# ParthaEth/GIF

Hardware: NVIDIA H100
Metric: G+D train step images/sec @256x256 bs32/GPU (higher is better)
Workload: dtype bf16x3 error-compensated tensor-core contraction (two-term bf16 operands, 3 MMAs per slice), f32 accumulate/storage

## Files before the change

### gif_b200/_lib.py

```python
import ctypes
import os

import torch

_HERE = os.path.dirname(os.path.abspath(__file__))
LIB_PATH = os.path.join(_HERE, "libgifb200.so")

_p = ctypes.c_void_p
_i = ctypes.c_int
_f = ctypes.c_float
_d = ctypes.c_double
_ll = ctypes.c_longlong
_sz = ctypes.c_size_t

SIGNATURES = {
    "gifb200_version": (_i, []),
    "gifb200_last_error": (ctypes.c_char_p, []),
    "gifb200_launch_count": (_ll, []),
    "gifb200_conv2d_workspace_bytes": (_sz, [_i] * 11),
    "gifb200_conv2d": (_i, [_p, _p, _p] + [_i] * 13 + [_p, _f, _f, _i, _p, _sz, _p]),
    "gifb200_conv2d_wgrad_workspace_bytes": (_sz, [_i] * 10),
    "gifb200_conv2d_wgrad_path": (_i, [_i] * 10),
    "gifb200_conv2d_wgrad": (_i, [_p, _p, _p] + [_i] * 12 + [_p, _sz, _p]),
    "gifb200_conv2d_ex_workspace_bytes": (_sz, [_i] * 13),
    "gifb200_conv2d_ex": (_i, [_p, _p, _p] + [_i] * 16 + [_p, _i, _p, _sz, _p]),
    "gifb200_pool2d": (_i, [_p, _p] + [_i] * 12 + [_p]),
    "gifb200_resize_bilinear": (_i, [_p, _p, _i, _i, _i, _ll, _ll, _ll, _ll, _i, _i, _i, _f, _f, _i, _p]),
    "gifb200_resize_bilinear_u8": (_i, [_p, _p, _i, _i, _i, _ll, _i, _i, _i, _f, _f, _i, _p]),
    "gifb200_split_bf16": (_i, [_p, _p, _p, _i, _i, _i, _p]),
    "gifb200_upfirdn2d": (_i, [_p, _p, _p] + [_i] * 14 + [_p]),
    "gifb200_bias_act": (_i, [_p, _p, _p, _p, _p, _i, _i, _i, _f, _f, _i, _p]),
    "gifb200_act_bwd": (_i, [_p, _p, _p, _ll, _f, _f, _i, _p]),
    "gifb200_rows_sum": (_i, [_p, _p, _i, _i, _i, _p]),
    "gifb200_chan_scale": (_i, [_p, _p, _p, _i, _i, _i, _i, _p]),
    "gifb200_tail_bwd": (_i, [_p] * 8 + [_i, _i, _i, _f, _f, _i, _p]),
    "gifb200_tail_bwd_planes": (_i, [_p] * 8 + [_i, _i, _i, _f, _f, _p, _p, _p]),
    "gifb200_scale_bwd": (_i, [_p] * 5 + [_i, _i, _i, _i, _p]),
    "gifb200_tail_bwd2": (_i, [_p] * 9 + [_i, _i, _i, _f, _f, _p, _p]),
    "gifb200_adam_step": (_i, [_p, _p, _p, _p, _p, _p, _i, _d, _d, _d, _d, _p]),
    "gifb200_spatial_dot": (_i, [_p, _p, _p, _i, _i, _i, _p]),
    "gifb200_axpby": (_i, [_p, _p, _p, _ll, _f, _f, _i, _p]),
    "gifb200_demod": (_i, [_p, _p, _p, _i, _i, _i, _f, _p]),
    "gifb200_torgb_fwd": (_i, [_p, _p, _p, _i, _i, _i, _p]),
    "gifb200_torgb_bwd_x": (_i, [_p, _p, _p, _i, _i, _i, _p]),
    "gifb200_torgb_bwd_w": (_i, [_p, _p, _p, _i, _i, _i, _p]),
    "gifb200_sgemm": (_i, [_i, _i, _i, _i, _i, _f, _p, _i, _p, _i, _p, _i, _p]),
    "gifb200_cond_down": (_i, [_p, _p, _i, _i, _i, _i, _i, _i, _p]),
    "gifb200_cond_up": (_i, [_p, _p, _i, _i, _i, _i, _i, _i, _p]),
    "gifb200_rasterize_workspace_bytes": (_sz, [_i, _i, _i, _i]),
    "gifb200_rasterize_fwd": (_i, [_p, _p, _p, _p, _p, _i, _i, _i, _i, _p, _sz, _p]),
    "gifb200_rasterize_fwd_ex": (_i, [_p] * 7 + [_i] * 5 + [_p, _sz, _p]),
    "gifb200_rasterize_bwd_ex": (_i, [_p] * 11 + [_i] * 5 + [_p]),
    "gifb200_render_shade": (_i, [_p] * 10 + [_i] * 5 + [_p]),
    "gifb200_vertex_normals": (_i, [_p] * 6 + [_i] * 3 + [_p]),
    "gifb200_rasterize_bwd": (_i, [_p, _p, _p, _p, _p, _p, _p, _p, _i, _i, _i, _i, _p]),
    "gifb200_flame_lbs_workspace_bytes": (_sz, [_i, _i]),
    "gifb200_flame_lbs": (_i, [_p] * 11 + [_i] * 4 + [_p, _sz, _p]),
    "gifb200_eye_camera": (_i, [_p, _p] + [_i] * 4 + [_f] * 4 + [_p]),
    "gifb200_flametex": (_i, [_p] * 4 + [_i] * 4 + [_p]),
    "gifb200_texture_steal_fwd": (_i, [_p] * 9 + [_i] * 6 + [_p]),
    "gifb200_texture_steal_bwd": (_i, [_p] * 7 + [_i] * 6 + [_p]),
    "gifb200_jpeg_workspace_bytes": (_sz, [_i, _i, _ll]),
    "gifb200_jpeg_decode": (_i, [_p] * 6 + [_i, _i, _i, _ll, _i, _i, _p, _p, _p, _sz, _p]),
    "gifb200_png_unfilter": (_i, [_p, _p, _i, _i, _p, _p, _p]),
    "gifb200_resize_bicubic_u8": (_i, [_p] * 5 + [_i] * 7 + [_p]),
    "gifb200_u8_to_unit": (_i, [_p, _p, _i, _i, _i, _ll, _p]),
    "gifb200_image_to_u8": (_i, [_p, _p, _i, _i, _i, _ll, _ll, _ll, _ll, _p]),
}


def _bind(path):
    lib = ctypes.CDLL(path)
    for name, (res, args) in SIGNATURES.items():
        fn = getattr(lib, name)
        fn.restype = res
        fn.argtypes = args
    return lib


def _load():
    import importlib.util
    spec = importlib.util.spec_from_file_location("_gifb200_build", os.path.join(_HERE, "build.py"))
# ... 39 lines not shown
```

### gif_b200/csrc/elementwise.cu

```cuda
#include <cuda_bf16.h>

#include <mutex>

#include "common.cuh"

namespace gifb200 {

thread_local char g_err[512] = "";
long long g_launches = 0;

template <bool VEC>
__global__ void __launch_bounds__(256) bias_act_kernel(const float* __restrict__ x, const float* __restrict__ rowscale,
                                                       const float* __restrict__ add, const float* __restrict__ bias,
                                                       float* __restrict__ y, long long total, int P, int C, float slope,
                                                       float gain, int rtf32) {
    const long long stride = static_cast<long long>(gridDim.x) * blockDim.x;
    if (VEC) {
        const long long nvec = total >> 2;
        const int c4n = C >> 2;
        for (long long v = static_cast<long long>(blockIdx.x) * blockDim.x + threadIdx.x; v < nvec; v += stride) {
            const int c = static_cast<int>(v % c4n) << 2;
            float4 t = __ldcs(reinterpret_cast<const float4*>(x) + v);
            if (rowscale) {
                const long long b = (v / c4n) / P;
// ... 374 lines not shown
                                                         float* __restrict__ y, long long total, int P, int C,
                                                         int rtf32) {
    const long long stride = static_cast<long long>(gridDim.x) * blockDim.x;
    if (VEC) {
        const long long nvec = total >> 2;
        const int c4n = C >> 2;
        for (long long v = static_cast<long long>(blockIdx.x) * blockDim.x + threadIdx.x; v < nvec; v += stride) {
            const int c = static_cast<int>(v % c4n) << 2;
            const long long b = (v / c4n) / P;
            float4 t = __ldcs(reinterpret_cast<const float4*>(x) + v);
            const float4 sc = *reinterpret_cast<const float4*>(s + b * C + c);
            t.x *= sc.x; t.y *= sc.y; t.z *= sc.z; t.w *= sc.w;
            if (rtf32) { t.x = round_tf32(t.x); t.y = round_tf32(t.y); t.z = round_tf32(t.z); t.w = round_tf32(t.w); }
            reinterpret_cast<float4*>(y)[v] = t;
        }
    } else {
        for (long long i = static_cast<long long>(blockIdx.x) * blockDim.x + threadIdx.x; i < total; i += stride) {
            float t = x[i] * s[((i / C) / P) * C + (i % C)];
            y[i] = rtf32 ? round_tf32(t) : t;
        }
    }
}


__global__ void __launch_bounds__(256) split_bf16_kernel(const float* __restrict__ x, const float* __restrict__ s,
                                                         __nv_bfloat16* __restrict__ planes, long long total, int P, int C) {
    const long long stride = static_cast<long long>(gridDim.x) * blockDim.x;
    const long long nvec = total >> 2;
    const int c4n = C >> 2;
    __nv_bfloat16* hi = planes;
    __nv_bfloat16* lo = planes + total;
    for (long long v = static_cast<long long>(blockIdx.x) * blockDim.x + threadIdx.x; v < nvec; v += stride) {
        float4 t = __ldcs(reinterpret_cast<const float4*>(x) + v);
        if (s) {
            const int c = static_cast<int>(v % c4n) << 2;
            const long long b = (v / c4n) / P;
            const float4 sc = *reinterpret_cast<const float4*>(s + b * C + c);
            t.x *= sc.x; t.y *= sc.y; t.z *= sc.z; t.w *= sc.w;
        }
        const __nv_bfloat16 h0 = __float2bfloat16_rn(t.x), h1 = __float2bfloat16_rn(t.y), h2 = __float2bfloat16_rn(t.z),
                            h3 = __float2bfloat16_rn(t.w);
        const __nv_bfloat16 l0 = __float2bfloat16_rn(t.x - __bfloat162float(h0)), l1 = __float2bfloat16_rn(t.y - __bfloat162float(h1)),
                            l2 = __float2bfloat16_rn(t.z - __bfloat162float(h2)), l3 = __float2bfloat16_rn(t.w - __bfloat162float(h3));
        uint2 ph, pl;
        ph.x = static_cast<uint32_t>(__bfloat16_as_ushort(h0)) | (static_cast<uint32_t>(__bfloat16_as_ushort(h1)) << 16);
        ph.y = static_cast<uint32_t>(__bfloat16_as_ushort(h2)) | (static_cast<uint32_t>(__bfloat16_as_ushort(h3)) << 16);
        pl.x = static_cast<uint32_t>(__bfloat16_as_ushort(l0)) | (static_cast<uint32_t>(__bfloat16_as_ushort(l1)) << 16);
        pl.y = static_cast<uint32_t>(__bfloat16_as_ushort(l2)) | (static_cast<uint32_t>(__bfloat16_as_ushort(l3)) << 16);
        reinterpret_cast<uint2*>(hi)[v] = ph;
        reinterpret_cast<uint2*>(lo)[v] = pl;
    }
}

template <bool VEC>
__global__ void __launch_bounds__(256) axpby_kernel(const float* __restrict__ a, const float* __restrict__ b,
                                                    float* __restrict__ y, long long n, float alpha, float beta,
                                                    int rtf32) {
    const long long stride = static_cast<long long>(gridDim.x) * blockDim.x;
    if (VEC) {
        const long long nvec = n >> 2;
        for (long long v = static_cast<long long>(blockIdx.x) * blockDim.x + threadIdx.x; v < nvec; v += stride) {
            float4 t = __ldcs(reinterpret_cast<const float4*>(a) + v);
            t.x *= alpha; t.y *= alpha; t.z *= alpha; t.w *= alpha;
            if (b) {
                const float4 u = __ldcs(reinterpret_cast<const float4*>(b) + v);
                t.x += beta * u.x; t.y += beta * u.y; t.z += beta * u.z; t.w += beta * u.w;
            }
            if (rtf32) { t.x = round_tf32(t.x); t.y = round_tf32(t.y); t.z = round_tf32(t.z); t.w = round_tf32(t.w); }
            reinterpret_cast<float4*>(y)[v] = t;
        }
    } else {
        for (long long i = static_cast<long long>(blockIdx.x) * blockDim.x + threadIdx.x; i < n; i += stride)
        {
            const float t = alpha * a[i] + (b ? beta * b[i] : 0.f);
            y[i] = rtf32 ? round_tf32(t) : t;
        }
    }
}

__global__ void __launch_bounds__(256) demod_kernel(const float* __restrict__ s, const float* __restrict__ q,
                                                    float* __restrict__ d, int B, int Ci, int Co, float eps) {
    const int warp = (blockIdx.x * blockDim.x + threadIdx.x) >> 5;
    const int lane = threadIdx.x & 31;
    if (warp >= B * Co) return;
    const int b = warp / Co, o = warp % Co;
    const float* sr = s + static_cast<long long>(b) * Ci;
    const float* qr = q + static_cast<long long>(o) * Ci;
    float acc = 0.f;
    for (int i = lane; i < Ci; i += 32) {
        const float sv = sr[i];
        acc += sv * sv * qr[i];
    }
    acc = warp_sum(acc);
    if (lane == 0) d[warp] = rsqrtf(acc + eps);
}

__global__ void __launch_bounds__(256) torgb_fwd_kernel(const float* __restrict__ x, const float* __restrict__ ws,
                                                        float* __restrict__ y, int B, int P, int C) {
    extern __shared__ float sw[];
    const int b = blockIdx.y;
    const float* wsb = ws + static_cast<long long>(b) * 3 * C;
    for (int i = threadIdx.x; i < 3 * C; i += blockDim.x) sw[i] = wsb[i];
    __syncthreads();
    const int warp = threadIdx.x >> 5, lane = threadIdx.x & 31, nwarp = blockDim.x >> 5;
    for (int p = blockIdx.x * nwarp + warp; p < P; p += gridDim.x * nwarp) {
        const float* xr = x + (static_cast<long long>(b) * P + p) * C;
// ... 520 lines not shown
    GIFB200_REQUIRE(!ggd || acc, GIFB200_E_SHAPE, "tail_bwd2: ggd needs acc");
    cudaStream_t st = static_cast<cudaStream_t>(stream);
    if (B == 0) return GIFB200_OK;
    if (gdd) {
        cudaError_t e = cudaMemsetAsync(gdd, 0, sizeof(float) * static_cast<size_t>(B) * C, st);
        if (e != cudaSuccess) return fail(GIFB200_E_CUDA, "tail_bwd2 memset", cudaGetErrorString(e));
    }
    if (P == 0) return GIFB200_OK;
    if (C % 32 == 0 && aligned16(gy) && (!gg || aligned16(gg)) && (!ggd || (aligned16(ggd) && aligned16(acc))) && (!y || aligned16(y)) &&
        (!d || aligned16(d)) && (!ggy || aligned16(ggy)) && (!gx2 || aligned16(gx2)) && (!gdd || aligned16(gdd)) &&
        (!ggy_planes || aligned16(ggy_planes))) {
        const int tx = vec_lanes(C);
        int rpb;
        const int cbv = C / (4 * tx);
        const int rb = rows_split_vec(P, cbv, B, 256 / tx, &rpb);
        GIFB200_REQUIRE(B <= 65535 && rb <= 65535, GIFB200_E_SHAPE, "tail_bwd2: grid too large");
        const dim3 grid(cbv, rb, B);
        Slots sl;
        if (int rc = gdd && gg ? slots_take(sl, gdd, rb, static_cast<long long>(B) * C, st) : GIFB200_OK) return rc;
        __nv_bfloat16* pp = static_cast<__nv_bfloat16*>(ggy_planes);
        const long long total = static_cast<long long>(B) * P * C;
        if (tx == 32) tail_bwd2_vec_kernel<32><<<grid, 256, 0, st>>>(gg, ggd, gy, y, acc, d, ggy, gx2, gdd, P, C, rpb, slope, gain, pp, total);
        else if (tx == 16) tail_bwd2_vec_kernel<16><<<grid, 256, 0, st>>>(gg, ggd, gy, y, acc, d, ggy, gx2, gdd, P, C, rpb, slope, gain, pp, total);
        else tail_bwd2_vec_kernel<8><<<grid, 256, 0, st>>>(gg, ggd, gy, y, acc, d, ggy, gx2, gdd, P, C, rpb, slope, gain, pp, total);
        GIFB200_LAUNCH_CHECK("tail_bwd2_vec_kernel");
        return sl.part ? slots_reduce(sl, st) : GIFB200_OK;
    }
    GIFB200_REQUIRE(!ggy_planes, GIFB200_E_ALIGN, "tail_bwd2: the planes output needs C % 32 == 0 and 16-byte aligned pointers");
    const int cb = cdiv(C, 32);
    int rpb;
    const int rb = rows_split(P, cb, B, &rpb);
    GIFB200_REQUIRE(B <= 65535 && rb <= 65535, GIFB200_E_SHAPE, "tail_bwd2: grid too large");
    Slots sl;
    if (int rc = gdd && gg ? slots_take(sl, gdd, rb, static_cast<long long>(B) * C, st) : GIFB200_OK) return rc;
    tail_bwd2_kernel<<<dim3(cb, rb, B), dim3(32, 8), 0, st>>>(gg, ggd, gy, y, acc, d, ggy, gx2, gdd, P, C, rpb, slope, gain);
    GIFB200_LAUNCH_CHECK("tail_bwd2_kernel");
    return sl.part ? slots_reduce(sl, st) : GIFB200_OK;
}

int gifb200_chan_scale(const float* x, const float* s, float* y, int B, int P, int C, int rtf32,
                       gifb200_stream_t stream) {
    GIFB200_REQUIRE(B >= 0 && P >= 0 && C > 0, GIFB200_E_SHAPE, "chan_scale: bad shape");
    const long long total = static_cast<long long>(B) * P * C;
    if (total == 0) return GIFB200_OK;
    cudaStream_t st = static_cast<cudaStream_t>(stream);
    if (C % 4 == 0 && aligned16(x) && aligned16(y) && aligned16(s))
        chan_scale_kernel<true><<<grid_for(total / 4, 256), 256, 0, st>>>(x, s, y, total, P, C, rtf32);
    else
        chan_scale_kernel<false><<<grid_for(total, 256), 256, 0, st>>>(x, s, y, total, P, C, rtf32);
    GIFB200_LAUNCH_CHECK("chan_scale_kernel");
    return GIFB200_OK;
}

int gifb200_split_bf16(const float* x, const float* s, void* planes, int B, int P, int C, gifb200_stream_t stream) {
    GIFB200_REQUIRE(B >= 0 && P >= 0 && C > 0 && C % 4 == 0, GIFB200_E_SHAPE, "split_bf16: C must be a positive multiple of 4");
    const long long total = static_cast<long long>(B) * P * C;
    if (total == 0) return GIFB200_OK;
    GIFB200_REQUIRE(aligned16(x) && aligned16(planes) && (!s || aligned16(s)), GIFB200_E_ALIGN, "split_bf16: pointers must be 16-byte aligned");
    split_bf16_kernel<<<grid_for(total / 4, 256), 256, 0, static_cast<cudaStream_t>(stream)>>>(
        x, s, static_cast<__nv_bfloat16*>(planes), total, P, C);
    GIFB200_LAUNCH_CHECK("split_bf16_kernel");
    return GIFB200_OK;
}

int gifb200_axpby(const float* a, const float* b, float* y, long long n, float alpha, float beta, int rtf32,
                  gifb200_stream_t stream) {
    if (n <= 0) return GIFB200_OK;
    cudaStream_t st = static_cast<cudaStream_t>(stream);
    if (n % 4 == 0 && aligned16(a) && aligned16(y) && (!b || aligned16(b)))
        axpby_kernel<true><<<grid_for(n / 4, 256), 256, 0, st>>>(a, b, y, n, alpha, beta, rtf32);
    else
        axpby_kernel<false><<<grid_for(n, 256), 256, 0, st>>>(a, b, y, n, alpha, beta, rtf32);
    GIFB200_LAUNCH_CHECK("axpby_kernel");
    return GIFB200_OK;
}

int gifb200_demod(const float* s, const float* q, float* d, int B, int Ci, int Co, float eps, gifb200_stream_t stream) {
    GIFB200_REQUIRE(B >= 0 && Ci > 0 && Co > 0, GIFB200_E_SHAPE, "demod: bad shape");
    if (B == 0) return GIFB200_OK;
    const long long warps = static_cast<long long>(B) * Co;
    demod_kernel<<<cdiv(warps * 32, 256), 256, 0, static_cast<cudaStream_t>(stream)>>>(s, q, d, B, Ci, Co, eps);
    GIFB200_LAUNCH_CHECK("demod_kernel");
    return GIFB200_OK;
}

int gifb200_torgb_fwd(const float* x, const float* ws, float* y, int B, int P, int C, gifb200_stream_t stream) {
    GIFB200_REQUIRE(B >= 0 && P >= 0 && C > 0 && C <= 4096, GIFB200_E_SHAPE, "torgb_fwd: bad shape");
    GIFB200_REQUIRE(B <= 65535, GIFB200_E_SHAPE, "torgb_fwd: batch too large");
    if (B == 0 || P == 0) return GIFB200_OK;
    GIFB200_REQUIRE(C % 4 != 0 || aligned16(x), GIFB200_E_ALIGN, "torgb_fwd: x not 16B aligned");
    if (C % 32 == 0 && aligned16(x) && aligned16(ws)) {
        const int tx = vec_lanes(C);
        int rpb;
        const int rb = rows_split_vec(P, 1, B, 256 / tx, &rpb);
        GIFB200_REQUIRE(rb <= 65535, GIFB200_E_SHAPE, "torgb_fwd: grid too large");
        const dim3 grid(1, rb, B);
        cudaStream_t st = static_cast<cudaStream_t>(stream);
        if (tx == 32) torgb_fwd_vec_kernel<32><<<grid, 256, 0, st>>>(x, ws, y, P, C, rpb);
        else if (tx == 16) torgb_fwd_vec_kernel<16><<<grid, 256, 0, st>>>(x, ws, y, P, C, rpb);
        else torgb_fwd_vec_kernel<8><<<grid, 256, 0, st>>>(x, ws, y, P, C, rpb);
        GIFB200_LAUNCH_CHECK("torgb_fwd_vec_kernel");
        return GIFB200_OK;
    }
    int gx = cdiv(P, 8 * 4);
    const int cap = max(1, kNumSMs * 8 / B);
    if (gx > cap) gx = cap;
// ... 95 lines not shown
```

### gif_b200/model/stg2_generator.py

```python
import random

import numpy as np
import torch
from torch import nn

from .. import ops
from .stylegan2_common_layers import StyledConv, ToRGB, get_w_frm_z


class ConstantInput(nn.Module):

    def __init__(self, channel, size=4, constant_background=False):
        super().__init__()
        self.input = nn.Parameter(torch.randn(1, channel, size, size))

    def forward(self, input):
        return self.input.repeat(input.shape[0], 1, 1, 1)


class ImgEmbedding(nn.Module):

    def __init__(self, vector_size, vocab_size=70_000):
        super().__init__()
        self.register_buffer('embd_weight', torch.randn((vocab_size, vector_size)))

    def get_embddings(self):
        return self.embd_weight

    def forward(self, input):
        return self.embd_weight[input]


class StyledConvStyleGAN2(nn.Module):

    def __init__(self, in_chnl, out_chnl, ker_sz, blur_kernel, noise_in_dims, one_conv_block=False,
                 apply_sqrt2_fac_in_eq_lin=False):
        super().__init__()
        self.one_conv_block = one_conv_block
        self.st_cv1 = StyledConv(in_chnl, out_chnl, ker_sz, upsample=not self.one_conv_block, blur_kernel=blur_kernel,
                                 noise_in_dims=noise_in_dims, apply_sqrt2_fac_in_eq_lin=apply_sqrt2_fac_in_eq_lin)
        if not self.one_conv_block:
            self.st_cv2 = StyledConv(out_chnl, out_chnl, ker_sz, upsample=False, blur_kernel=blur_kernel,
                                     noise_in_dims=noise_in_dims, apply_sqrt2_fac_in_eq_lin=apply_sqrt2_fac_in_eq_lin)

    def forward_nhwc(self, x, style, noise_nhwc):
        x = self.st_cv1.forward_nhwc(x, style, noise_nhwc)
        if self.one_conv_block:
            return x
        return self.st_cv2.forward_nhwc(x, style, noise_nhwc)

    def forward(self, input, style, noise=None):
        n = None if noise is None else ops.to_nhwc(noise)
        return ops.to_nchw_view(self.forward_nhwc(ops.to_nhwc(input), style, n))


class Generator(nn.Module):

    def __init__(self, code_dim, core_tensor_res=4, channel_multiplier=2, noise_in_dims=None,
                 apply_sqrt2_fac_in_eq_lin=False):
        super().__init__()
        assert core_tensor_res < 64
        assert code_dim == 512
        m = channel_multiplier
        self.start_step = int(np.log2(core_tensor_res)) - 2
        self.const_input = ConstantInput(512, size=core_tensor_res)
        blur_kernel = [1, 3, 3, 1]
        chans = [512, 512, 512, 512, 256 * m, 128 * m, 64 * m, 32 * m, 16 * m]
        kw = dict(blur_kernel=blur_kernel, noise_in_dims=noise_in_dims,
                  apply_sqrt2_fac_in_eq_lin=apply_sqrt2_fac_in_eq_lin)
        blocks = [StyledConvStyleGAN2(code_dim, chans[0], 3, one_conv_block=True, **kw)]
        for i in range(1, 9):
            blocks.append(StyledConvStyleGAN2(chans[i - 1], chans[i], 3, **kw))
        self.progression = nn.ModuleList(blocks)
        self.to_rgb = nn.ModuleList(
            [ToRGB(chans[i], code_dim, upsample=i > 0, apply_sqrt2_fac_in_eq_lin=apply_sqrt2_fac_in_eq_lin)
             for i in range(9)])

    def forward(self, style, pose, noise, step=0, alpha=-1, input_indices=None, mixing_range=(-1, -1)):
        out = torch.zeros((noise[0].shape[0], 3), device=noise[0].device) if pose is None else pose
        if len(style) < 2:
            inject_index = [len(self.progression) + 1]
        else:
            inject_index = random.sample(list(range(step)), len(style) - 1)
        crossover = 0
        rgb = None
        x = None
        for i in range(self.start_step, len(self.progression)):
            if mixing_range == (-1, -1):
                if crossover < len(inject_index) and i > inject_index[crossover]:
                    crossover = min(crossover + 1, len(style))
                style_step = style[crossover]
            else:
                style_step = style[1] if mixing_range[0] <= i <= mixing_range[1] else style[0]
            if i == self.start_step:
                x = ops.to_nhwc(self.const_input(out))
            x = self.progression[i].forward_nhwc(x, style_step, ops.to_nhwc(noise[i]))
            rgb = self.to_rgb[i].forward_nhwc(x, style_step, rgb)
            if i == step:
                break
        return [ops.to_nchw_view(rgb)]


# ... 66 lines not shown
```

### gif_b200/model/stylegan2_common_layers.py

```python
import math
import random

import torch
from torch import nn
from torch.nn import functional as F

from .. import ops


def make_kernel(k):
    k = torch.tensor(k, dtype=torch.float32)
    if k.ndim == 1:
        k = k[None, :] * k[:, None]
    k /= k.sum()
    return k


def upfirdn2d(input, kernel, up=1, down=1, pad=(0, 0)):
    return ops.to_nchw_view(ops.upfirdn2d(ops.to_nhwc(input), kernel, up=up, down=down, pad=pad))


class FusedLeakyReLU(nn.Module):

    def __init__(self, channel, negative_slope=0.2, scale=2 ** 0.5):
# ... 17 lines not shown
    def __init__(self, kernel, factor=2):
        super().__init__()
        self.factor = factor
        kernel = make_kernel(kernel) * (factor ** 2)
        self.register_buffer('kernel', kernel)
        p = kernel.shape[0] - factor
        self.pad = ((p + 1) // 2 + factor - 1, p // 2)

    def forward(self, input):
        return upfirdn2d(input, self.kernel, up=self.factor, down=1, pad=self.pad)


class Downsample(nn.Module):

    def __init__(self, kernel, factor=2):
        super().__init__()
        self.factor = factor
        kernel = make_kernel(kernel)
        self.register_buffer('kernel', kernel)
        p = kernel.shape[0] - factor
        self.pad = ((p + 1) // 2, p // 2)

    def forward(self, input):
        return upfirdn2d(input, self.kernel, up=1, down=self.factor, pad=self.pad)


class Blur(nn.Module):

    def __init__(self, kernel, pad, upsample_factor=1):
        super().__init__()
        kernel = make_kernel(kernel)
        if upsample_factor > 1:
            kernel = kernel * (upsample_factor ** 2)
        self.register_buffer('kernel', kernel)
        self.pad = pad

    def forward(self, input):
        return upfirdn2d(input, self.kernel, pad=self.pad)


def _conv_mode(kernel_size, stride, padding):
    if stride == 1 and padding == kernel_size // 2:
        return ops.S1
    if stride == 2 and padding == 0:
        return ops.S2
    raise NotImplementedError(f"gif_b200 convolution: (k={kernel_size}, stride={stride}, padding={padding}) is not on "
                              "the GIF hot path (supported: stride 1 with 'same' padding, stride 2 without padding)")


def _pad_channels_for_tc(x, wt):
    ci = x.shape[-1]
    if ops.tc_enabled() and ci % 32 != 0 and wt.shape[1] % 32 == 0:
        pad = 32 - ci % 32
        x = F.pad(x, (0, pad))
        wt = F.pad(wt, (0, pad))
    return x, wt


class EqualConv2d(nn.Module):

    def __init__(self, in_channel, out_channel, kernel_size, stride=1, padding=0, bias=True):
        super().__init__()
        self.weight = nn.Parameter(torch.randn(out_channel, in_channel, kernel_size, kernel_size))
        self.scale = 1 / math.sqrt(in_channel * kernel_size ** 2)
        self.stride = stride
        self.padding = padding
        self.kernel_size = kernel_size
        self.bias = nn.Parameter(torch.zeros(out_channel)) if bias else None

    def forward_nhwc(self, x):
        mode = _conv_mode(self.kernel_size, self.stride, self.padding)
        wt = ops.prep_weight(self.weight, self.scale, cache=self.training)
        x, wt = _pad_channels_for_tc(x, wt)
        if self.bias is not None:
            return ops.conv2d_bias_act(x, wt, self.bias, self.kernel_size, mode, slope=1.0, gain=1.0)
        return ops.conv2d(x, wt, self.kernel_size, mode)

    def forward(self, input):
        return ops.to_nchw_view(self.forward_nhwc(ops.to_nhwc(input)))

    def __repr__(self):
        return (f'{self.__class__.__name__}({self.weight.shape[1]}, {self.weight.shape[0]},'
                f' {self.weight.shape[2]}, stride={self.stride}, padding={self.padding})')


class EqualLinear(nn.Module):

    def __init__(self, in_dim, out_dim, bias=True, bias_init=0, lr_mul=1, activation=None, scale_weight=1.0,
                 apply_sqrt2_fac_in_eq_lin=False):
        super().__init__()
        self.weight = nn.Parameter(torch.randn(out_dim, in_dim).div_(lr_mul / scale_weight))
        self.bias = nn.Parameter(torch.zeros(out_dim).fill_(bias_init)) if bias else None
        self.activation = activation
        self.scale = (1 / math.sqrt(in_dim)) * lr_mul
        self.lr_mul = lr_mul
        self.apply_sqrt2_fac_in_eq_lin = apply_sqrt2_fac_in_eq_lin

    def forward(self, input):
        x = input.reshape(-1, input.shape[-1])
        y = ops.matmul(x, self.weight, trans_b=True, alpha=self.scale)
        bias = None if self.bias is None else self.bias * self.lr_mul
        if self.activation:
            gain = 1.41421356237 if self.apply_sqrt2_fac_in_eq_lin else 1.0
            y = ops.bias_act(y, bias, slope=0.2, gain=gain)
        elif bias is not None:
            y = ops.bias_act(y, bias, slope=1.0, gain=1.0)
        return y.reshape(input.shape[:-1] + (self.weight.shape[0],))
# ... 45 lines not shown

    def accumulate(self, x, style):
        s = self.modulation(style)
        wt = ops.prep_weight(self.weight[0], self.scale, cache=self.training)
        k = self.kernel_size
        if k == 1 and self.out_channel == 3 and not (self.upsample or self.downsample):
            acc = ops.torgb(x, wt[0][None] * s[:, None, :])
        else:
            if self.upsample:
                acc = ops.modconv(x, s, wt, k, ops.T2)
                acc = ops.upfirdn2d(acc, self.blur.kernel, pad=self.blur.pad)
            elif self.downsample:
                xs = ops.chan_scale(x, s, ops.tf32_enabled())
                xs = ops.upfirdn2d(xs, self.blur.kernel, pad=self.blur.pad, rt=ops.tf32_enabled())
                acc = ops.conv2d(xs, wt, k, ops.S2)
            else:
                acc = ops.modconv(x, s, wt, k, ops.S1)
        d = None
        if self.demodulate:
            q = (wt * wt).sum(dim=0)
            d = ops.demod(s, q, self.eps)
        return acc, d

    def forward_nhwc(self, x, style):
        acc, d = self.accumulate(x, style)
        return acc if d is None else ops.chan_scale(acc, d)

    def forward(self, input, style):
        return ops.to_nchw_view(self.forward_nhwc(ops.to_nhwc(input), style))


class NoiseInjection(nn.Module):

    @staticmethod
    def small_init_weights(m):
        if hasattr(m, 'weight'):
            m.weight.data = torch.randn_like(m.weight) / 100
        if hasattr(m, 'bias'):
            m.bias.data.fill_(0.0001)

    def __init__(self, noise_in_chalnnels, noise_out_channels):
        super().__init__()
        self.noise_in_chalnnels = noise_in_chalnnels
        c = noise_in_chalnnels
        self.noise_conv = nn.Sequential(
            nn.Conv2d(in_channels=c, out_channels=2 * c, kernel_size=3, padding=1, dilation=1),
            nn.ReLU(),
            nn.Conv2d(in_channels=2 * c, out_channels=4 * c, kernel_size=3, padding=1, dilation=1),
            nn.ReLU(),
            nn.Conv2d(in_channels=4 * c, out_channels=noise_out_channels, kernel_size=3, padding=1, dilation=1),
        )
        self.noise_conv.apply(NoiseInjection.small_init_weights)

    def convolved_noise_nhwc(self, noise):
        c0, c2, c4 = self.noise_conv[0], self.noise_conv[2], self.noise_conv[4]
        w0, w2, w4 = (ops.prep_weight(c.weight, cache=self.training) for c in (c0, c2, c4))
        b0, b2 = c0.bias, c2.bias
        if ops.tc_enabled() and noise.shape[1] >= 4 and (noise.shape[1] & (noise.shape[1] - 1)) == 0:
            def up32(n):
                return (n + 31) // 32 * 32
            ci, c1, c2n = w0.shape[2], w0.shape[1], w2.shape[1]
            noise = F.pad(noise, (0, up32(ci) - ci))
            w0 = F.pad(w0, (0, up32(ci) - ci, 0, up32(c1) - c1))
            b0 = F.pad(b0, (0, up32(c1) - c1))
            w2 = F.pad(w2, (0, up32(c1) - c1, 0, up32(c2n) - c2n))
            b2 = F.pad(b2, (0, up32(c2n) - c2n))
            w4 = F.pad(w4, (0, up32(c2n) - c2n))
        rt = ops.tf32_enabled()
        h = ops.conv2d_bias_act(noise, w0, b0, 3, ops.S1, slope=0.0, gain=1.0, rt=rt)
        h = ops.conv2d_bias_act(h, w2, b2, 3, ops.S1, slope=0.0, gain=1.0, rt=rt)
        h = ops.conv2d(h, w4, 3, ops.S1)
        return h, c4.bias

    def forward(self, image, noise):
        x = ops.to_nhwc(image)
        if noise is None:
            b, _, hh, ww = image.shape
            noise = image.new_empty(b, self.noise_in_chalnnels, hh, ww).normal_()
        h, b4 = self.convolved_noise_nhwc(ops.to_nhwc(noise))
        return ops.to_nchw_view(ops.bias_act(h, b4, slope=1.0, gain=1.0, add=x))


class ConstantInput(nn.Module):

    def __init__(self, channel, size=4):
        super().__init__()
        self.input = nn.Parameter(torch.randn(1, channel, size, size))

    def forward(self, input):
        return self.input.repeat(input.shape[0], 1, 1, 1)


class StyledConv(nn.Module):

    def __init__(self, in_channel, out_channel, kernel_size, noise_in_dims, style_dim=512, upsample=False,
                 blur_kernel=[1, 3, 3, 1], demodulate=True, apply_sqrt2_fac_in_eq_lin=False):
        super().__init__()
        self.conv = ModulatedConv2d(in_channel, out_channel, kernel_size, style_dim, upsample=upsample,
                                    blur_kernel=blur_kernel, demodulate=demodulate,
                                    apply_sqrt2_fac_in_eq_lin=apply_sqrt2_fac_in_eq_lin)
        self.noise = NoiseInjection(noise_in_dims, out_channel)
        self.activate = FusedLeakyReLU(out_channel)

    def forward_nhwc(self, x, style, noise_nhwc):
        acc, d = self.conv.accumulate(x, style)
        if noise_nhwc is None:
            b, hh, ww, _ = acc.shape
            noise_nhwc = acc.new_empty(b, hh, ww, self.noise.noise_in_chalnnels).normal_()
        h, b4 = self.noise.convolved_noise_nhwc(noise_nhwc)
        bias = self.activate.bias.reshape(-1) + b4
        return ops.bias_act(acc, bias, self.activate.negative_slope, self.activate.scale, rowscale=d, add=h)

    def forward(self, input, style, noise=None):
        n = None if noise is None else ops.to_nhwc(noise)
        return ops.to_nchw_view(self.forward_nhwc(ops.to_nhwc(input), style, n))


class ToRGB(nn.Module):

    def __init__(self, in_channel, style_dim, upsample=True, blur_kernel=[1, 3, 3, 1],
                 apply_sqrt2_fac_in_eq_lin=False):
        super().__init__()
        if upsample:
            self.upsample = Upsample(blur_kernel)
        self.conv = ModulatedConv2d(in_channel, 3, 1, style_dim, demodulate=False,
                                    apply_sqrt2_fac_in_eq_lin=apply_sqrt2_fac_in_eq_lin)
        self.bias = nn.Parameter(torch.zeros(1, 3, 1, 1))

    def forward_nhwc(self, x, style, skip):
        acc, _ = self.conv.accumulate(x, style)
        if skip is not None:
            skip = ops.upfirdn2d(skip, self.upsample.kernel, up=self.upsample.factor, pad=self.upsample.pad)
        return ops.bias_act(acc, self.bias, slope=1.0, gain=1.0, add=skip)

    def forward(self, input, style, skip=None):
        s = None if skip is None else ops.to_nhwc(skip)
        return ops.to_nchw_view(self.forward_nhwc(ops.to_nhwc(input), style, s))


def get_w_frm_z(n_mlp, style_dim, lr_mlp=1, scale_weight=1.0):
    if n_mlp > 0:
        layers = [PixelNorm()]
        for _ in range(n_mlp):
            layers.append(EqualLinear(style_dim, style_dim, lr_mul=lr_mlp, activation='fused_lrelu',
                                      scale_weight=scale_weight))
        return nn.Sequential(*layers)

    class Net(nn.Module):
        def forward(self, *args):
            return args[0]

    return Net()


class Generator(nn.Module):

    def __init__(self, size, style_dim, n_mlp, channel_multiplier=2, blur_kernel=[1, 3, 3, 1], lr_mlp=0.01):
        super().__init__()
        self.size = size
        self.style_dim = style_dim
        self.style = get_w_frm_z(n_mlp, style_dim, lr_mlp)
        m = channel_multiplier
# ... 129 lines not shown
```

### gif_b200/ops.py

```python
import math
import os
import weakref

import torch

from ._lib import GifB200Error, check, lib, ptr, require_cuda, stream

S1, S2, T2 = 0, 1, 2
_ADJ_MODE = {S1: S1, S2: T2, T2: S2}
CONV_IMPL = 0
WGRAD_IMPL = 0
_PRECISION = "tf32"


_WEIGHT_GRADS = [True]


class input_gradient_only:

    def __enter__(self):
        self.prev = _WEIGHT_GRADS[0]
        _WEIGHT_GRADS[0] = False

    def __exit__(self, *a):
        _WEIGHT_GRADS[0] = self.prev
        return False


def set_precision(mode):
    global CONV_IMPL, _PRECISION
    if mode not in ("tf32", "bf16x3", "fp32"):
        raise ValueError(mode)
    _PRECISION = mode
    CONV_IMPL = {"tf32": 0, "bf16x3": 3, "fp32": 1}[mode]


def get_precision():
    return _PRECISION


def tf32_enabled():
    return _PRECISION == "tf32" and CONV_IMPL != 1


def tc_enabled():
    return _PRECISION in ("tf32", "bf16x3") and CONV_IMPL != 1


def _planes(x):
    c = getattr(x, "_gifb200_planes", None)
    if c is not None and c[0] == x._version:
        return c[1]
    B, C = x.shape[0], x.shape[-1]
    P = x.numel() // max(B * C, 1)
    pl = torch.empty((2,) + tuple(x.shape), dtype=torch.bfloat16, device=x.device)
    check(lib.gifb200_split_bf16(ptr(x), None, ptr(pl), B, P, C, stream()), "gifb200_split_bf16")
    x._gifb200_planes = (x._version, pl)
    return pl


def _carry_planes(x, planes):
    if planes is not None:
        x._gifb200_planes = (x._version, planes)


def _tag(t, rounded):
    if rounded:
        t._gifb200_tf32 = t._version
    return t


def _is_tf32(t):
    return getattr(t, "_gifb200_tf32", None) == t._version


def _round_tf32_raw(x):
    y = torch.empty_like(x)
    check(lib.gifb200_axpby(ptr(x), None, ptr(y), x.numel(), 1.0, 0.0, 1, stream()), "gifb200_axpby(round)")
    return y

PROFILE = None

_ws_cache = {}
_ws_retired = []


def _workspace(nbytes, device):
    if nbytes == 0:
        return None
    key = (device.index, torch.cuda.current_stream().cuda_stream)
    buf = _ws_cache.get(key)
    if buf is None or buf.numel() < nbytes:
        if buf is not None:
            _ws_retired.append(buf)
        buf = torch.empty(max(nbytes, 1 << 20), dtype=torch.uint8, device=device)
        _ws_cache[key] = buf
    return buf


def _c(t):
    return t if t.is_contiguous() else t.contiguous()


def conv_out_size(hi, k, mode):
    if mode == S1:
        return hi
    if mode == S2:
        return (hi - k) // 2 + 1
    return 2 * (hi - 1) + k


# ... 952 lines not shown
```

### include/gifb200.h

```cpp
#ifndef GIFB200_H
#define GIFB200_H

#include <stddef.h>
#include <stdint.h>

#ifdef __cplusplus
extern "C" {
#endif

#define GIFB200_OK 0
#define GIFB200_E_SHAPE (-1)
#define GIFB200_E_ALIGN (-2)
#define GIFB200_E_ARCH (-3)
#define GIFB200_E_CUDA (-4)
#define GIFB200_E_WORKSPACE (-5)

typedef void* gifb200_stream_t;

int gifb200_version(void);
const char* gifb200_last_error(void);
long long gifb200_launch_count(void);

#define GIFB200_CONV_PRESTAGED 0x10
size_t gifb200_conv2d_workspace_bytes(int B, int Hi, int Wi, int Ci, int Ho, int Wo, int Co, int k, int mode,
                                      int transposed, int impl);
int gifb200_conv2d(const float* x, const float* w, float* y, int B, int Hi, int Wi, int Ci, int Ho, int Wo, int Co,
                   int k, int mode, int flip, int transposed, int impl, int act, const float* bias, float slope,
                   float gain, int round_tf32, void* workspace, size_t workspace_bytes, gifb200_stream_t stream);

size_t gifb200_conv2d_wgrad_workspace_bytes(int B, int Hi, int Wi, int Ci, int Ho, int Wo, int Co, int k, int mode,
                                            int impl);
int gifb200_conv2d_wgrad_path(int B, int Hi, int Wi, int Ci, int Ho, int Wo, int Co, int k, int mode, int impl);
int gifb200_conv2d_wgrad(const float* x, const float* gy, float* gw, int B, int Hi, int Wi, int Ci, int Ho, int Wo,
                         int Co, int k, int mode, int flip, int transposed, int impl, void* workspace,
                         size_t workspace_bytes, gifb200_stream_t stream);

size_t gifb200_conv2d_ex_workspace_bytes(int B, int Hi, int Wi, int Ci, int Ho, int Wo, int Co, int kh, int kw, int stride,
                                         int pad_h, int pad_w, int impl);
int gifb200_conv2d_ex(const void* x, const float* w, float* y, int B, int Hi, int Wi, int Ci, int Ho, int Wo, int Co, int kh,
                      int kw, int stride, int pad_h, int pad_w, int Cy, int c0, int impl, int act, const float* bias,
                      int round_tf32, void* workspace, size_t workspace_bytes, gifb200_stream_t stream);
int gifb200_pool2d(const float* x, float* y, int B, int Hi, int Wi, int C, int Ho, int Wo, int stride, int pad, int op, int Cy,
                   int c0, int round_tf32, gifb200_stream_t stream);
int gifb200_resize_bilinear(const float* x, float* y, int B, int H, int W, long long stride_b, long long stride_c,
                            long long stride_h, long long stride_w, int Ho, int Wo, int Cy, float scale, float shift,
                            int round_tf32, gifb200_stream_t stream);
int gifb200_resize_bilinear_u8(const uint8_t* x, float* y, int B, int H, int W, long long stride_b, int Ho, int Wo, int Cy,
                               float scale, float shift, int round_tf32, gifb200_stream_t stream);

int gifb200_split_bf16(const float* x, const float* s, void* planes, int B, int P, int C, gifb200_stream_t stream);

int gifb200_upfirdn2d(const float* x, const float* kernel, float* y, int B, int Hi, int Wi, int C, int Ho, int Wo,
                      int kh, int kw, int up, int down, int pad_y0, int pad_x0, int flip, int round_tf32,
                      gifb200_stream_t stream);

int gifb200_bias_act(const float* x, const float* rowscale, const float* add, const float* bias, float* y, int B,
                     int P, int C, float slope, float gain, int round_tf32, gifb200_stream_t stream);
int gifb200_act_bwd(const float* gy, const float* y, float* gx, long long n, float slope, float gain,
                    int round_tf32, gifb200_stream_t stream);
int gifb200_rows_sum(const float* x, float* out, int G, int rows, int C, gifb200_stream_t stream);
int gifb200_chan_scale(const float* x, const float* s, float* y, int B, int P, int C, int round_tf32,
                       gifb200_stream_t stream);
int gifb200_tail_bwd(const float* gy, const float* y, const float* acc, const float* d, float* gt, float* gacc, float* gb,
                     float* gd, int B, int P, int C, float slope, float gain, int round_tf32, gifb200_stream_t stream);
int gifb200_scale_bwd(const float* gy, const float* x, const float* s, float* gx, float* gs, int B, int P, int C,
                      int round_tf32, gifb200_stream_t stream);
int gifb200_tail_bwd_planes(const float* gy, const float* y, const float* acc, const float* d, float* gt, float* gacc,
                            float* gb, float* gd, int B, int P, int C, float slope, float gain, void* gt_planes,
                            void* gacc_planes, gifb200_stream_t stream);
int gifb200_tail_bwd2(const float* gg, const float* ggd, const float* gy, const float* y, const float* acc, const float* d,
                      float* ggy, float* gx2, float* gdd, int B, int P, int C, float slope, float gain, void* ggy_planes,
                      gifb200_stream_t stream);
int gifb200_adam_step(float* const* params, const float* const* grads, float* const* exp_avg, float* const* exp_avg_sq,
                      float* const* steps, const long long* numel, int count, double lr, double beta1, double beta2, double eps,
                      gifb200_stream_t stream);
int gifb200_spatial_dot(const float* a, const float* b2, float* out, int B, int P, int C, gifb200_stream_t stream);
int gifb200_axpby(const float* a, const float* b, float* y, long long n, float alpha, float beta, int round_tf32,
                  gifb200_stream_t stream);
int gifb200_demod(const float* s, const float* q, float* d, int B, int Ci, int Co, float eps, gifb200_stream_t stream);

int gifb200_torgb_fwd(const float* x, const float* ws, float* y, int B, int P, int C, gifb200_stream_t stream);
int gifb200_torgb_bwd_x(const float* gy, const float* ws, float* gx, int B, int P, int C, gifb200_stream_t stream);
int gifb200_torgb_bwd_w(const float* gy, const float* x, float* gws, int B, int P, int C, gifb200_stream_t stream);

int gifb200_sgemm(int transA, int transB, int M, int N, int K, float alpha, const float* A, int lda, const float* B,
                  int ldb, float* C, int ldc, gifb200_stream_t stream);

int gifb200_cond_down(float* x, float* y, int B, int H, int W, int C, int s, int adjoint,
                      gifb200_stream_t stream);
int gifb200_cond_up(float* x, float* y, int B, int H, int W, int C, int s, int adjoint,
                    gifb200_stream_t stream);

size_t gifb200_rasterize_workspace_bytes(int B, int F, int h, int w);
int gifb200_rasterize_fwd(const float* face_vertices, const float* face_colors, float* depth, int32_t* triangle,
                          float* out3, int B, int F, int h, int w, void* workspace, size_t workspace_bytes,
                          gifb200_stream_t stream);
int gifb200_rasterize_fwd_ex(const float* face_vertices, const float* face_colors, const float* face_colors2, float* depth,
                             int32_t* triangle, float* out3, float* out3b, int B, int F, int h, int w, int convention,
                             void* workspace, size_t workspace_bytes, gifb200_stream_t stream);
int gifb200_rasterize_bwd(const float* face_vertices, const float* face_colors, const int32_t* triangle,
                          const float* g_bary, const float* g_img, const float* g_depth, float* g_face_vertices,
                          float* g_face_colors, int B, int F, int h, int w, gifb200_stream_t stream);
int gifb200_rasterize_bwd_ex(const float* face_vertices, const float* face_colors, const float* face_colors2,
// ... 56 lines not shown
```

Baseline: 82.33.

## Fuse channel padding with bf16 split and share padded noise across convs

Adds a pad_channels kernel that zero-pads the channel dimension and, in the same pass, writes the hi/lo bf16 planes used by the bf16x3 tensor-core conv, then attaches those planes to the padded tensor. This replaces F.pad plus a separate split pass. The styled block also pads the noise once and reuses it for both convs instead of padding it per conv. The new kernel is scalar and uses a per-element integer division, and correctness depends on the attached planes staying valid for the reused padded tensor.

```diff
diff --git a/gif_b200/_lib.py b/gif_b200/_lib.py
--- a/gif_b200/_lib.py
+++ b/gif_b200/_lib.py
@@ -28,6 +28,7 @@
     "gifb200_resize_bilinear": (_i, [_p, _p, _i, _i, _i, _ll, _ll, _ll, _ll, _i, _i, _i, _f, _f, _i, _p]),
     "gifb200_resize_bilinear_u8": (_i, [_p, _p, _i, _i, _i, _ll, _i, _i, _i, _f, _f, _i, _p]),
     "gifb200_split_bf16": (_i, [_p, _p, _p, _i, _i, _i, _p]),
+    "gifb200_pad_channels": (_i, [_p, _p, _p, _ll, _i, _i, _p]),
     "gifb200_upfirdn2d": (_i, [_p, _p, _p] + [_i] * 14 + [_p]),
     "gifb200_bias_act": (_i, [_p, _p, _p, _p, _p, _i, _i, _i, _f, _f, _i, _p]),
     "gifb200_act_bwd": (_i, [_p, _p, _p, _ll, _f, _f, _i, _p]),
diff --git a/gif_b200/csrc/elementwise.cu b/gif_b200/csrc/elementwise.cu
--- a/gif_b200/csrc/elementwise.cu
+++ b/gif_b200/csrc/elementwise.cu
@@ -450,6 +450,22 @@
     }
 }
 
+__global__ void __launch_bounds__(256) pad_channels_kernel(const float* __restrict__ x, float* __restrict__ y,
+                                                           __nv_bfloat16* __restrict__ planes, long long total, int C, int Cp) {
+    const long long stride = static_cast<long long>(gridDim.x) * blockDim.x;
+    for (long long e = static_cast<long long>(blockIdx.x) * blockDim.x + threadIdx.x; e < total; e += stride) {
+        const long long r = e / Cp;
+        const int c = static_cast<int>(e - r * Cp);
+        const float v = c < C ? __ldg(x + r * C + c) : 0.f;
+        y[e] = v;
+        if (planes) {
+            const __nv_bfloat16 h = __float2bfloat16_rn(v);
+            planes[e] = h;
+            planes[total + e] = __float2bfloat16_rn(v - __bfloat162float(h));
+        }
+    }
+}
+
 template <bool VEC>
 __global__ void __launch_bounds__(256) axpby_kernel(const float* __restrict__ a, const float* __restrict__ b,
                                                     float* __restrict__ y, long long n, float alpha, float beta,
@@ -1076,6 +1092,16 @@
     return GIFB200_OK;
 }
 
+int gifb200_pad_channels(const float* x, float* y, void* planes, long long rows, int C, int Cp, gifb200_stream_t stream) {
+    GIFB200_REQUIRE(rows >= 0 && C > 0 && Cp >= C, GIFB200_E_SHAPE, "pad_channels: bad shape");
+    const long long total = rows * Cp;
+    if (total == 0) return GIFB200_OK;
+    pad_channels_kernel<<<grid_for(total, 256), 256, 0, static_cast<cudaStream_t>(stream)>>>(
+        x, y, static_cast<__nv_bfloat16*>(planes), total, C, Cp);
+    GIFB200_LAUNCH_CHECK("pad_channels_kernel");
+    return GIFB200_OK;
+}
+
 int gifb200_split_bf16(const float* x, const float* s, void* planes, int B, int P, int C, gifb200_stream_t stream) {
     GIFB200_REQUIRE(B >= 0 && P >= 0 && C > 0 && C % 4 == 0, GIFB200_E_SHAPE, "split_bf16: C must be a positive multiple of 4");
     const long long total = static_cast<long long>(B) * P * C;
diff --git a/gif_b200/model/stg2_generator.py b/gif_b200/model/stg2_generator.py
--- a/gif_b200/model/stg2_generator.py
+++ b/gif_b200/model/stg2_generator.py
@@ -44,10 +44,11 @@
                                      noise_in_dims=noise_in_dims, apply_sqrt2_fac_in_eq_lin=apply_sqrt2_fac_in_eq_lin)
 
     def forward_nhwc(self, x, style, noise_nhwc):
-        x = self.st_cv1.forward_nhwc(x, style, noise_nhwc)
+        padded = None if noise_nhwc is None else self.st_cv1.noise.padded_noise(noise_nhwc)
+        x = self.st_cv1.forward_nhwc(x, style, noise_nhwc, padded)
         if self.one_conv_block:
             return x
-        return self.st_cv2.forward_nhwc(x, style, noise_nhwc)
+        return self.st_cv2.forward_nhwc(x, style, noise_nhwc, padded)
 
     def forward(self, input, style, noise=None):
         n = None if noise is None else ops.to_nhwc(noise)
diff --git a/gif_b200/model/stylegan2_common_layers.py b/gif_b200/model/stylegan2_common_layers.py
--- a/gif_b200/model/stylegan2_common_layers.py
+++ b/gif_b200/model/stylegan2_common_layers.py
@@ -93,7 +93,7 @@
     ci = x.shape[-1]
     if ops.tc_enabled() and ci % 32 != 0 and wt.shape[1] % 32 == 0:
         pad = 32 - ci % 32
-        x = F.pad(x, (0, pad))
+        x = ops.pad_channels(x, ci + pad)
         wt = F.pad(wt, (0, pad))
     return x, wt
 
@@ -245,15 +245,23 @@
         )
         self.noise_conv.apply(NoiseInjection.small_init_weights)
 
-    def convolved_noise_nhwc(self, noise):
+    @staticmethod
+    def padded_noise(noise):
+        if ops.tc_enabled() and noise.shape[1] >= 4 and (noise.shape[1] & (noise.shape[1] - 1)) == 0:
+            return ops.pad_channels(noise, (noise.shape[-1] + 31) // 32 * 32)
+        return None
+
+    def convolved_noise_nhwc(self, noise, padded=None):
         c0, c2, c4 = self.noise_conv[0], self.noise_conv[2], self.noise_conv[4]
         w0, w2, w4 = (ops.prep_weight(c.weight, cache=self.training) for c in (c0, c2, c4))
         b0, b2 = c0.bias, c2.bias
-        if ops.tc_enabled() and noise.shape[1] >= 4 and (noise.shape[1] & (noise.shape[1] - 1)) == 0:
+        if padded is None:
+            padded = self.padded_noise(noise)
+        if padded is not None:
             def up32(n):
                 return (n + 31) // 32 * 32
             ci, c1, c2n = w0.shape[2], w0.shape[1], w2.shape[1]
-            noise = F.pad(noise, (0, up32(ci) - ci))
+            noise = padded
             w0 = F.pad(w0, (0, up32(ci) - ci, 0, up32(c1) - c1))
             b0 = F.pad(b0, (0, up32(c1) - c1))
             w2 = F.pad(w2, (0, up32(c1) - c1, 0, up32(c2n) - c2n))
@@ -295,12 +303,12 @@
         self.noise = NoiseInjection(noise_in_dims, out_channel)
         self.activate = FusedLeakyReLU(out_channel)
 
-    def forward_nhwc(self, x, style, noise_nhwc):
+    def forward_nhwc(self, x, style, noise_nhwc, padded_noise=None):
         acc, d = self.conv.accumulate(x, style)
         if noise_nhwc is None:
             b, hh, ww, _ = acc.shape
             noise_nhwc = acc.new_empty(b, hh, ww, self.noise.noise_in_chalnnels).normal_()
-        h, b4 = self.noise.convolved_noise_nhwc(noise_nhwc)
+        h, b4 = self.noise.convolved_noise_nhwc(noise_nhwc, padded_noise)
         bias = self.activate.bias.reshape(-1) + b4
         return ops.bias_act(acc, bias, self.activate.negative_slope, self.activate.scale, rowscale=d, add=h)
 
diff --git a/gif_b200/ops.py b/gif_b200/ops.py
--- a/gif_b200/ops.py
+++ b/gif_b200/ops.py
@@ -57,6 +57,33 @@
     check(lib.gifb200_split_bf16(ptr(x), None, ptr(pl), B, P, C, stream()), "gifb200_split_bf16")
     x._gifb200_planes = (x._version, pl)
     return pl
+
+
+class _PadChannels(torch.autograd.Function):
+
+    @staticmethod
+    def forward(ctx, x, cp):
+        x = _c(x)
+        require_cuda(x)
+        c = x.shape[-1]
+        y = torch.empty(tuple(x.shape[:-1]) + (cp,), dtype=torch.float32, device=x.device)
+        pl = torch.empty((2,) + tuple(y.shape), dtype=torch.bfloat16, device=x.device) if CONV_IMPL == 3 else None
+        check(lib.gifb200_pad_channels(ptr(x), ptr(y), ptr(pl), x.numel() // max(c, 1), c, cp, stream()),
+              "gifb200_pad_channels")
+        ctx.c = c
+        if pl is not None:
+            ctx.mark_non_differentiable(pl)
+        return y, pl
+
+    @staticmethod
+    def backward(ctx, g, _):
+        return g[..., :ctx.c], None
+
+
+def pad_channels(x, cp):
+    y, pl = _PadChannels.apply(x, cp)
+    _carry_planes(y, pl)
+    return y
 
 
 def _carry_planes(x, planes):
diff --git a/include/gifb200.h b/include/gifb200.h
--- a/include/gifb200.h
+++ b/include/gifb200.h
@@ -49,6 +49,7 @@
                                float scale, float shift, int round_tf32, gifb200_stream_t stream);
 
 int gifb200_split_bf16(const float* x, const float* s, void* planes, int B, int P, int C, gifb200_stream_t stream);
+int gifb200_pad_channels(const float* x, float* y, void* planes, long long rows, int C, int Cp, gifb200_stream_t stream);
 
 int gifb200_upfirdn2d(const float* x, const float* kernel, float* y, int B, int Hi, int Wi, int C, int Ho, int Wo,
                       int kh, int kw, int up, int down, int pad_y0, int pad_x0, int flip, int round_tf32,
```

After: 82.60, median of 6. About the same (+0.3%).
